# 54rt1n/shardmerge

Measured on AMD Instinct MI355X. Metric: merged-weight GB/s per GPU + % HBM roofline, Llama-3-70B 3-way FFT merge, higher is better.
Workload: dtype f32; 1 GPU; Llama-3-70B block tensors, this rank's 1/8 slice (9 per block x 10 blocks), K=3 finetunes, bf16 in/out, resident in HBM; workload_id=llama3-70b-slice, k=3, parallelism=tensor-partition x1 (no data-path collective), streams_per_gpu=8

## Files before the change

### shardmerge_amd/csrc/fft_engine.hpp

```cpp
#pragma once
#include <cmath>
#include <cstdint>
#include <type_traits>

#if defined(__HIPCC__)
#include <hip/hip_runtime.h>
#define SM_HD __host__ __device__ __forceinline__
#else
#define SM_HD inline
#endif
#define SM_CONST static constexpr
#if defined(__HIP_DEVICE_COMPILE__)
#define SM_OPAQUE(x) asm volatile("" : "+v"(x))
#else
#define SM_OPAQUE(x) ((void)0)
#endif
#if defined(__HIP_DEVICE_COMPILE__)
#define SM_LAUNDER(x) asm("" : "+v"(x))
#else
#define SM_LAUNDER(x) ((void)0)
#endif
#if defined(__HIP_DEVICE_COMPILE__) && !defined(SM_NO_SCHED_BARRIER)
#define SM_SCHED_FENCE() __builtin_amdgcn_sched_barrier(0)
#else
#define SM_SCHED_FENCE() ((void)0)
#endif

namespace smhip {

#include "twiddle_consts.inc"

constexpr int EMAX = 32;
constexpr int EREG = EMAX + 4;
constexpr int MAX_PASSES = 8;

struct cf2 { float x, y; };

#if defined(__HIP_DEVICE_COMPILE__)
typedef float vf2 __attribute__((ext_vector_type(2)));
SM_HD vf2 mk2(float a, float b) { vf2 v; v.x = a; v.y = b; return v; }
#else
struct vf2 { float x, y; };
SM_HD vf2 mk2(float a, float b) { vf2 v; v.x = a; v.y = b; return v; }
SM_HD vf2 operator+(vf2 a, vf2 b) { return mk2(a.x + b.x, a.y + b.y); }
SM_HD vf2 operator-(vf2 a, vf2 b) { return mk2(a.x - b.x, a.y - b.y); }
SM_HD vf2 operator*(vf2 a, vf2 b) { return mk2(a.x * b.x, a.y * b.y); }
SM_HD vf2 operator*(vf2 a, float b) { return mk2(a.x * b, a.y * b); }
SM_HD vf2 operator*(float a, vf2 b) { return mk2(a * b.x, a * b.y); }
SM_HD vf2 operator-(vf2 a) { return mk2(-a.x, -a.y); }
SM_HD vf2& operator+=(vf2& a, vf2 b) { a = a + b; return a; }
#endif

struct FftPlanDev {
    int N;
    int T;
    int npass;
    int radix[MAX_PASSES];
    const cf2* tw;
    int lds_floats;
    int cx;
};

template <int I, int N, class F>
SM_HD void static_for(F&& f) {
    if constexpr (I < N) {
        f(std::integral_constant<int, I>{});
        static_for<I + 1, N>(f);
    }
// ... 661 lines not shown
```

### shardmerge_amd/csrc/sm_capi.inc

```

struct smhip_ctx {
    smhip::Pipeline<SM_BACKEND> pipe;
    explicit smhip_ctx(int device) : pipe(device) {}
};

#define SM_GUARD(ctx)                      \
    if (!(ctx)) return SMHIP_ERR_ARG;      \
    (ctx)->pipe.err.clear();
#define SM_FINISH(ctx, rc)                                                        \
    do {                                                                          \
        int rc__ = (rc);                                                          \
        if (rc__ == SMHIP_OK && !(ctx)->pipe.be.ok()) {                           \
            (ctx)->pipe.err = (ctx)->pipe.be.error();                             \
            rc__ = SMHIP_ERR_HIP;                                                 \
        }                                                                         \
        return rc__;                                                              \
    } while (0)

template <class Desc, class Scalars>
static int delta_tensor_check(smhip_ctx* ctx, const char* op, const Desc* d, const void* out, const float* delta_out,
                              bool need_base, Scalars scalars) {
    auto bad = [&](const char* what) { return ctx->pipe.fail(SMHIP_ERR_ARG, std::string(op) + ": " + what); };
    if (!d) return bad("null descriptor");
    if (d->k < 1 || d->k > SMHIP_MAX_MODELS) return bad("k out of range (1..16)");
// ... 703 lines not shown
    SM_GUARD(ctx);
    if (!norm_out || (n > 0 && !x)) return ctx->pipe.fail(SMHIP_ERR_ARG, "bad argument");
    if (dtype < SMHIP_BF16 || dtype > SMHIP_F32) return ctx->pipe.fail(SMHIP_ERR_ARG, "bad dtype");
    ctx->pipe.stream = stream;
    SM_FINISH(ctx, ctx->pipe.fn_exact_norm(x, dtype, n, norm_out));
}

int smhip_correlate_pairs(smhip_ctx* ctx, int k, const void* const* tensors, int dtype, size_t rows, size_t cols,
                          float* matrix_out, void* stream) {
    SM_GUARD(ctx);
    if (!tensors || !matrix_out || rows < 1 || cols < 1) return ctx->pipe.fail(SMHIP_ERR_ARG, "bad argument");
    if (dtype < SMHIP_BF16 || dtype > SMHIP_F32) return ctx->pipe.fail(SMHIP_ERR_ARG, "bad dtype");
    for (int i = 0; i < k && i < 8; ++i)
        if (!tensors[i]) return ctx->pipe.fail(SMHIP_ERR_ARG, "null tensor");
    ctx->pipe.stream = stream;
    SM_FINISH(ctx, ctx->pipe.correlate_pairs(k, tensors, dtype, rows, cols, matrix_out));
}

int smhip_reference_cpu_norm(smhip_ctx* ctx, const void* x, const void* base, int dtype, size_t n, float* norm_out,
                             void* stream) {
    SM_GUARD(ctx);
    if (!x || !norm_out) return ctx->pipe.fail(SMHIP_ERR_ARG, "bad argument");
    if (dtype < SMHIP_BF16 || dtype > SMHIP_F32) return ctx->pipe.fail(SMHIP_ERR_ARG, "bad dtype");
    ctx->pipe.stream = stream;
    const int rc0 = ctx->pipe.reserve(1, 1);
    if (rc0) SM_FINISH(ctx, rc0);
    smhip::SigDesc sg{x, base, dtype, 1.f};
    double out = 0;
    if (!ctx->pipe.run_serial_norms(&sg, 1, n, &out))
        return ctx->pipe.fail(SMHIP_ERR_ARG, "reference_cpu norm: inputs must be 16-byte aligned");
    *norm_out = (float)out;
    SM_FINISH(ctx, SMHIP_OK);
}

int smhip_debug_option(smhip_ctx* ctx, const char* key, long value) {
    SM_GUARD(ctx);
    if (key && std::string(key) == "aten_overlap") { ctx->pipe.aten_overlap = value != 0; return SMHIP_OK; }
    if (key && std::string(key) == "emf_max_sample") { ctx->pipe.emf_max_sample = value >= 1 && value <= 4096 ? (int)value : smhip::EMF_MAX_SAMPLE; return SMHIP_OK; }
    if (key && std::string(key) == "aten_serial") { ctx->pipe.aten_serial = value != 0; return SMHIP_OK; }
    if (key && std::string(key) == "class_norms") { ctx->pipe.class_norms_mode = value >= 0 && value <= 2 ? (int)value : 1; return SMHIP_OK; }
    if (key && std::string(key) == "cand_cap") { ctx->pipe.debug_cand_cap = value > 0 ? (uint32_t)value : 0u; return SMHIP_OK; }
    if (key && std::string(key) == "sel_chunks") { ctx->pipe.debug_sel_chunks = value > 0 ? (uint32_t)value : 0u; return SMHIP_OK; }
    if (key && std::string(key) == "sel_flush_always") { ctx->pipe.debug_flush_always = value != 0; return SMHIP_OK; }
    if (key && std::string(key) == "fuse_norms") { ctx->pipe.fuse_norms = value != 0; return SMHIP_OK; }
    if (key && std::string(key) == "noise_seed") { ctx->pipe.noise_seed_base = (uint32_t)value; return SMHIP_OK; }
    if (key && std::string(key) == "spectral_intermediates") { ctx->pipe.spectral_inter = value != 0; return SMHIP_OK; }
    if (key && std::string(key) == "fuse_spec_norm") { ctx->pipe.fuse_spec_norm = value != 0; return SMHIP_OK; }
    if (key && std::string(key) == "sel_wgs_per_cu") { ctx->pipe.sel_wgs_per_cu = value > 0 ? (int)value : 5; return SMHIP_OK; }
    if (key && std::string(key) == "pair1d") { ctx->pipe.pair1d_enabled = value != 0; return SMHIP_OK; }
    if (key && std::string(key) == "spec_cull") { ctx->pipe.spec_cull = value != 0; return SMHIP_OK; }
    if (key && std::string(key) == "spec_min_bins") { ctx->pipe.spec_min_bins = value >= 0 ? (size_t)value : (size_t)1 << 20; return SMHIP_OK; }
    if (key && std::string(key) == "dftp_pairs") { ctx->pipe.dftp_pairs_enabled = value != 0; return SMHIP_OK; }
    if (key && std::string(key) == "f2s_pair") { ctx->pipe.f2s_pair = value != 0; return SMHIP_OK; }
    if (key && std::string(key) == "f1_multi") { ctx->pipe.f1_multi = value != 0; return SMHIP_OK; }
    if (key && std::string(key) == "force_bluestein") { ctx->pipe.debug_force_bluestein = value != 0; return SMHIP_OK; }
    if (key && std::string(key) == "force_split") { ctx->pipe.debug_force_split = value > 1 && value <= smhip::DFTP_MAX_P ? (int)value : 0; return SMHIP_OK; }
    if (key && std::string(key) == "fold_columns") { ctx->pipe.fold_enabled = value != 0; return SMHIP_OK; }
    if (key && std::string(key) == "della_slab_rows") { ctx->pipe.delta.della_slab_rows = value > 0 ? (size_t)value : 0; return SMHIP_OK; }
    if (key && std::string(key) == "fold_min_rows") { ctx->pipe.fold_min_rows = value > 0 ? (int)value : SM_FOLD_MIN_ROWS; return SMHIP_OK; }
    return ctx->pipe.fail(SMHIP_ERR_ARG, "unknown debug option");
}

int smhip_debug_query(smhip_ctx* ctx, const char* key, long* value) {
    SM_GUARD(ctx);
    if (!key || !value) return SMHIP_ERR_ARG;
    if (std::string(key) == "spec_hit") { *value = ctx->pipe.last_spec_verdict(); SM_FINISH(ctx, SMHIP_OK); }
    if (std::string(key) == "spec_checked" || std::string(key) == "spec_hits") {
        unsigned long long c = 0, h = 0;
        ctx->pipe.spec_totals(&c, &h);
        *value = (long)(std::string(key) == "spec_hits" ? h : c);
        SM_FINISH(ctx, SMHIP_OK);
    }
    if (std::string(key) == "aten_fast" || std::string(key) == "aten_group" || std::string(key) == "aten_slow") {
        unsigned long long v3[3];
        ctx->pipe.aten_stats(1, v3);
        *value = (long)v3[std::string(key) == "aten_fast" ? 0 : std::string(key) == "aten_group" ? 1 : 2];
        SM_FINISH(ctx, SMHIP_OK);
    }
    if (std::string(key) == "eig_host_us") { *value = (long)ctx->pipe.delta.eig_host_us; SM_FINISH(ctx, SMHIP_OK); }
    return ctx->pipe.fail(SMHIP_ERR_ARG, "unknown debug query");
}

int smhip_profile_enable(smhip_ctx* ctx, int on) { SM_GUARD(ctx); ctx->pipe.be.profile_enable(on != 0); return SMHIP_OK; }
int smhip_profile_reset(smhip_ctx* ctx) { SM_GUARD(ctx); ctx->pipe.be.profile_reset(); return SMHIP_OK; }
int smhip_profile_count(smhip_ctx* ctx) { return ctx ? ctx->pipe.be.profile_count() : 0; }
int smhip_profile_get(smhip_ctx* ctx, int i, const char** name, uint64_t* launches, double* total_ms) {
    SM_GUARD(ctx);
    return ctx->pipe.be.profile_get(i, name, launches, total_ms) ? SMHIP_OK : SMHIP_ERR_ARG;
}

}
```

### shardmerge_amd/csrc/sm_kernels.hpp

```cpp
#pragma once
#include <cmath>
#include <cstring>

#include "fft_engine.hpp"
#include "sm_aten_core.hpp"

namespace smhip {

struct cf4 { float x, y, z, w; };
struct u32x4 { uint32_t x, y, z, w; };

enum { DT_BF16 = 0, DT_F16 = 1, DT_F32 = 2 };

struct SigDesc {
    const void* x;
    const void* base;
    int dtype;
    float prescale;
};

SM_HD uint32_t umax(uint32_t a, uint32_t b) { return a > b ? a : b; }
SM_HD float u2f(uint32_t u) { float f; memcpy(&f, &u, 4); return f; }
SM_HD uint32_t f2u(float f) { uint32_t u; memcpy(&u, &f, 4); return u; }
SM_HD float bf16_to_f(uint32_t h) { return u2f(h << 16); }
// ... 620 lines not shown
                Dft<4>::run(ar, ai);
                Dft<4>::run(br, bi);
#pragma unroll
                for (int k1 = 0; k1 < 4; ++k1) {
                    if (k1) {
                        const cf2 wa = p.twR[(size_t)n2A * k1], wb = p.twR[(size_t)n2B * k1];
                        cmul(ar[k1], ai[k1], wa.x, wa.y); cmul(br[k1], bi[k1], wb.x, wb.y);
                    }
                    cf4 v = {ar[k1], ai[k1], br[k1], bi[k1]};
                    if (live) rowp[(size_t)k * p.ilv + k1 * slabstride] = v;
                }
                SM_SCHED_FENCE();
            };
#pragma unroll
            for (int jj = 0; jj < NJ; ++jj) {
                const int u = 4 * jj + g;
                if (u < E2) {
                    const int k = t + u * T;
                    const int k2 = (k == 0) ? 0 : C - k;
                    float aim[4], bre[4];
#pragma unroll
                    for (int gp = 0; gp < 4; ++gp) {
                        const float* l = lds + gp * LF;
                        const float v1 = l[lpad(k)], v2 = l[lpad(k2)];
                        const int sl = (jj * 4 + gp) * 2;
                        if (comp == 0) { s.xr[sl] = 0.5f * (v1 + v2); s.xr[sl + 1] = 0.5f * (v2 - v1); }
                        else           { aim[gp] = 0.5f * (v1 - v2); bre[gp] = 0.5f * (v1 + v2); }
                    }
                    if (comp == 1) {
                        float are[4], bim[4];
#pragma unroll
                        for (int gp = 0; gp < 4; ++gp) { are[gp] = s.xr[(jj * 4 + gp) * 2]; bim[gp] = s.xr[(jj * 4 + gp) * 2 + 1]; }
                        emit(k, are, aim, bre, bim);
                    }
                }
            }
            if (tid == 0) {
                if (comp == 0) {
#pragma unroll
                    for (int gp = 0; gp < 4; ++gp) s.xr[NJ * 8 + gp] = lds[gp * LF + lpad(C / 2)];
                } else {
                    float are[4], aim[4] = {0.f, 0.f, 0.f, 0.f}, bre[4], bim[4] = {0.f, 0.f, 0.f, 0.f};
#pragma unroll
                    for (int gp = 0; gp < 4; ++gp) { are[gp] = s.xr[NJ * 8 + gp]; bre[gp] = lds[gp * LF + lpad(C / 2)]; }
                    emit(C / 2, are, aim, bre, bim);
                }
            }
        });

    ex.template block_sum<2>(st, [&](const double* tot) {
        partials_[2 * (size_t)pbid] = tot[0];
        partials_[2 * (size_t)pbid + 1] = tot[1];
    });
    }
}

struct SliceGrid { int wgs = 0; size_t t1_stride = 0, plane_stride = 0; };
template <class Ex> SM_HD int slice_of(Ex& ex, const SliceGrid& sl, int& bid) {
    bid = ex.bid();
    if (sl.wgs <= 0) return 0;
    const int s = bid / sl.wgs;
    bid -= s * sl.wgs;
    return s;
}

struct F2Params {
    FftPlanDev plan;
    const cf4* t1;
    int pitch4;
    int ilv;
    int R, C, Cb;
    int nsig;
    int swap;
    float scale[2];
    float* reA; float* imA; float* reB;
    unsigned long long* hist;
    int slab;
    int Cb_real;
    int Rfull;
    size_t slab_elems;
    SliceGrid sl;
};
SM_HD int fold_bin(int v, int slab, int Cb_real, int R2, int Rfull, size_t& off) {
    const int k1 = v / slab, k = v % slab;
    off = (size_t)k * Rfull + (size_t)k1 * R2;
    return k < Cb_real ? k : -1;
}

#ifndef SM_T1_ILV
#define SM_T1_ILV 2
#endif
#ifndef SM_T1_ILV_MIN_ROWS
#define SM_T1_ILV_MIN_ROWS 8192
#endif
#ifndef SM_F2_MAX_THREADS
#define SM_F2_MAX_THREADS 512
#endif
SM_HD constexpr int t1_interleave_rows(int R) { return R >= SM_T1_ILV_MIN_ROWS ? SM_T1_ILV : 1; }
SM_HD constexpr int f2_nsig_for(int T) { return (2 * T <= SM_F2_MAX_THREADS) ? 2 : 1; }

constexpr int FOLD_ILV = 2;
template <class P> constexpr bool fold_col_plan() {
    if constexpr (P::is_static) return f2_nsig_for(P::T) == 2 && (P::N == 2048 || P::N == 3584 || P::N == 4096 || P::N == 7168);
    else return false;
}
template <class P, int BINS, bool FOLD = false, class Ex>
// ... 3167 lines not shown
```

### shardmerge_amd/csrc/sm_pipeline.hpp

```cpp
#pragma once
#include <algorithm>
#include <cmath>
#include <cstdio>
#include <map>
#include <string>
#include <vector>

#include "../../include/shardmerge_hip.h"
#include "sm_kernels.hpp"
#include "sm_aten_norm.hpp"
#include "sm_bluestein.hpp"
#include "sm_lora.hpp"
#include "sm_delta_host.hpp"

namespace smhip {

#define SM_KERNEL_TAG(Tag, ParamsT, NAME, CALL)                                      \
    struct Tag {                                                                     \
        using Params = ParamsT;                                                      \
        static constexpr int waves = 4;                                              \
        static constexpr int max_threads = 1024;                                     \
        static const char* name() { return NAME; }                                   \
        template <class Ex> static SM_HD void run(Ex& ex, const Params& p) { CALL; } \
    };
template <class P, int GROUPS> constexpr int fft_max_threads() {
    if constexpr (P::is_static) return (GROUPS * P::T < 256) ? 256 : (GROUPS * P::T > 1024 ? 1024 : GROUPS * P::T);
    else return 1024;
}
#ifndef SM_W3_MAX_THREADS
#define SM_W3_MAX_THREADS 256
#endif
#define SM_FFT_KERNEL_TAG(Tag, ParamsT, NAME, CALL, GROUPS, WAVES)                   \
    template <class P> struct Tag {                                                  \
        using Params = ParamsT;                                                      \
        static constexpr int waves = (WAVES < 4 && P::is_static && fft_max_threads<P, GROUPS>() <= SM_W3_MAX_THREADS) ? WAVES : 4; \
        static constexpr int max_threads = waves < 4 ? fft_max_threads<P, GROUPS>() : 1024; \
        static const char* name() { return NAME; }                                   \
        template <class Ex> static SM_HD void run(Ex& ex, const Params& p) { CALL; } \
    };
SM_FFT_KERNEL_TAG(KF1, F1Params, "f1_rows_fwd", k_f1<P>(ex, p), 1, 3)
SM_FFT_KERNEL_TAG(KF2, F2Params, "f2_cols_fwd", (k_f2<P, f2_bins<P>()>(ex, p)), 2 * f2_bins<P>(), 4)
SM_FFT_KERNEL_TAG(KI1x1, I1Params, "i1_cols_inv", (k_i1<P, 1>(ex, p)), 1, 4)
SM_FFT_KERNEL_TAG(KI1x2, I1Params, "i1_cols_inv", (k_i1<P, i1_bins<P>()>(ex, p)), i1_bins<P>(), 4)
SM_FFT_KERNEL_TAG(KI2, I2Params, "i2_rows_inv", k_i2<P>(ex, p), 1, 4)
SM_FFT_KERNEL_TAG(KF2S, F2SParams, "f2s_cols_fwd1", (k_f2s<P, f2s_groups<P>()>(ex, p)), f2s_groups<P>(), 4)
SM_FFT_KERNEL_TAG(KF1Q, F1Params, "f1_rows_fwd", k_f1q<P>(ex, p), 4, 4)
SM_FFT_KERNEL_TAG(KF2Q, F2Params, "f2_cols_fwd", (k_f2<P, f2_bins<P>(), true>(ex, p)), 2 * f2_bins<P>(), 4)
SM_FFT_KERNEL_TAG(KF2SQ, F2SParams, "f2s_cols_fwd1", (k_f2s<P, f2s_groups<P>(), true>(ex, p)), f2s_groups<P>(), 4)
SM_FFT_KERNEL_TAG(KI1x1Q, I1Params, "i1_cols_inv", (k_i1<P, 1, true>(ex, p)), 1, 4)
SM_FFT_KERNEL_TAG(KI1x2Q, I1Params, "i1_cols_inv", (k_i1<P, i1_bins<P>(), true>(ex, p)), i1_bins<P>(), 4)
#define SM_BLUE_KERNEL_TAG(Tag, ParamsT, NAME, CALL)                                 \
    template <class P> struct Tag {                                                  \
        using Params = ParamsT;                                                      \
        static constexpr int max_threads = fft_max_threads<P, 1>();                  \
        static constexpr int waves = max_threads > 512 ? 4 : 2;                      \
        static const char* name() { return NAME; }                                   \
        template <class Ex> static SM_HD void run(Ex& ex, const Params& p) { CALL; } \
    };
SM_BLUE_KERNEL_TAG(KF1B, F1BParams, "f1_rows_fwd", k_f1b<P>(ex, p))
SM_BLUE_KERNEL_TAG(KI2B, I2BParams, "i2_rows_inv", k_i2b<P>(ex, p))
SM_FFT_KERNEL_TAG(KPair1d, Pair1dParams, "pair_1d", k_pair1d<P>(ex, p), 1, 1)

#ifndef SM_COLS_MAX_THREADS
#define SM_COLS_MAX_THREADS 1024
#endif
#ifndef SM_F2_MAX_THREADS
#define SM_F2_MAX_THREADS 512
#endif
#ifndef SM_R14336
#define SM_R14336 16, 16, 8, 7
#endif
#ifndef SM_R7168
#define SM_R7168 32, 32, 7
#endif
#ifndef SM_T8192
#define SM_T8192 256
#define SM_W8192 4
#define SM_R8192 32, 16, 16
#endif
#define SM_STATIC_PLANS(X)                 \
    X(SPlan<1024, 64, false, 4, 32, 32>)       \
    X(SPlan<2048, 64, false, 4, 16, 16, 8>)    \
    X(SPlan<4096, 128, false, 4, 16, 16, 16>)  \
    X(SPlan<8192, SM_T8192, false, SM_W8192, SM_R8192>)  \
    X(SPlan<16384, 512, false, 4, 32, 32, 16>)\
    X(SPlan<14336, 512, false, 4, SM_R14336>) \
    X(SPlan<28672, 1024, false, 4, 16, 16, 16, 7>) \
    X(SPlan<3072, 128, false, 4, 16, 16, 4, 3>)    \
    X(SPlan<3584, 128, false, 4, 16, 32, 7>)       \
    X(SPlan<5120, 256, false, 4, 16, 16, 4, 5>)    \
    X(SPlan<6144, 256, false, 4, 16, 16, 8, 3>)    \
    X(SPlan<7168, 256, false, 4, SM_R7168>)    \
    X(SPlan<12288, 512, false, 4, 16, 16, 16, 3>)  \
    X(SPlan<13824, 512, false, 4, 32, 16, 3, 3, 3>) \
    X(SPlan<27648, 1024, false, 4, 32, 32, 3, 3, 3>) \
    X(SPlan<2304, 128, false, 4, 16, 16, 3, 3>) \
    X(SPlan<256, 64, false, 4, 8, 8, 4>)            \
    X(SPlan<512, 64, false, 4, 32, 16>)             \
    X(SPlan<64, 64, false, 4, 8, 8>)                \
// ... 147 lines not shown
        if (N % p) continue;
        M = N / p;
        if (M % 2 == 0 && plan_shape(M, T, rad)) return true;
    }
    return false;
}
inline int bluestein_len(int C) {
    if (C < 2) return 0;
    for (int L = 256; L <= EMAX * 1024; L *= 2)
        if (L >= 2 * C - 1) return L;
    return 0;
}
inline int shape_support(int rows, int cols, bool* transposed = nullptr) {
    int T, p, M;
    std::vector<int> rad;
    if (transposed) *transposed = false;
    if (rows < 1 || cols < 1) return 0;
    if (plan_shape(cols, T, rad) && rough_split(rows, p, M)) return 1;
    if (plan_shape(rows, T, rad) && rough_split(cols, p, M)) { if (transposed) *transposed = true; return 1; }
    if (bluestein_len(cols) && rough_split(rows, p, M)) return 1;
    if (bluestein_len(rows) && rough_split(cols, p, M)) { if (transposed) *transposed = true; return 1; }
    return 0;
}

struct ProfEntry { std::string name; uint64_t launches = 0; double ms = 0; };

struct PairOut {
    void* out = nullptr; int out_mode = OUT_F32;
    const void* base = nullptr; int base_dtype = DT_BF16;
    float post = 1.f;
    int ifft_policy = 1;
};

template <class B>
class Pipeline {
  public:
    B be;
    std::string err;
    void* stream = nullptr;
    DeltaHost<B> delta{be, err, stream};
    uint32_t debug_cand_cap = 0;
    uint32_t debug_sel_chunks = 0;
    bool debug_flush_always = false;
    bool spec_cull = true;
    size_t spec_min_bins = 1 << 20;
    bool dftp_pairs_enabled = true;
    int debug_force_split = 0;
    int sel_wgs_per_cu = 5;
    bool safe_select = false;
    uint32_t noise_seed_base = 0;
    bool spectral_inter = true;
    bool f2s_pair = true;
    size_t f2s_pair_max_bins = (size_t)64 << 20;
    bool f1_multi = true;
    bool fuse_spec_norm = true;
    float noise_sigma = 1.2e-7f;

    explicit Pipeline(int device) : be(device) {}
    ~Pipeline() {
        for (auto& kv : plans_) if (kv.second.dev.tw) be.free((void*)kv.second.dev.tw);
        for (Buffer* b : {&cand_, &t1_, &small_, &tmpA_, &tmpB_, &tmpC_, &fullS_, &saveR_, &saveI_, &aten_, &emf_, &lora_, &dora_}) if (b->p) be.free(b->p);
        for (Buffer& b : pool_) if (b.p) be.free(b.p);
        if (mail_) be.free_host(mail_);
        for (Buffer& b : inter_) if (b.p) be.free(b.p);
        for (Buffer& b : rowspec_) if (b.p) be.free(b.p);
        for (Buffer& b : tr_) if (b.p) be.free(b.p);
        for (auto& kv : rough_tw_) if (kv.second) be.free(kv.second);
        for (auto& kv : blue_) { if (kv.second.chirp) be.free(kv.second.chirp); if (kv.second.filt) be.free(kv.second.filt); }
    }

    int fail(int code, const std::string& msg) { err = msg; return code; }

    int get_plan(int N, FftPlanDev& out) {
        auto it = plans_.find(N);
        if (it == plans_.end()) {
            HostPlan hp;
            int T;
            std::vector<int> rad;
            if (plan_shape(N, T, rad)) {
                hp.ok = true;
                hp.dev.N = N; hp.dev.T = T; hp.dev.npass = (int)rad.size();
                for (int i = 0; i < MAX_PASSES; ++i) hp.dev.radix[i] = i < (int)rad.size() ? rad[i] : 1;
                hp.dev.cx = plan_uses_cx(N) ? 1 : 0;
                hp.dev.lds_floats = hp.dev.cx ? (int)round_up((size_t)2 * (N + (N >> 4) + 1), 32)
                                              : (int)round_up((size_t)lpad(N) + 1, 32);
                std::vector<cf2> tw(N);
                for (int j = 0; j < N; ++j) {
                    const double ang = -2.0 * M_PI * (double)j / (double)N;
                    tw[j].x = (float)cos(ang); tw[j].y = (float)sin(ang);
                }
                void* d = be.alloc(sizeof(cf2) * N);
                if (!d) return fail(SMHIP_ERR_NOMEM, "twiddle alloc failed");
                be.h2d(d, tw.data(), sizeof(cf2) * N, stream);
                hp.dev.tw = (const cf2*)d;
            } else {
                hp.dev.tw = nullptr;
            }
            it = plans_.emplace(N, hp).first;
        }
        if (!it->second.ok) {
            char buf[256];
            snprintf(buf, sizeof buf, "unsupported transform length %d (a row length needs factors in {2,3,5,7,11,13} and <= %d; the layer merge "
                                       "also takes p * M column lengths, p <= %d)", N, EMAX * 1024, DFTP_MAX_P);
            return fail(SMHIP_ERR_SHAPE, buf);
        }
        out = it->second.dev;
// ... 201 lines not shown
            bh.filt = be.alloc(sizeof(cf2) * L);
            if (!bh.chirp || !bh.filt) return fail(SMHIP_ERR_NOMEM, "chirp table alloc failed");
            be.h2d(bh.chirp, chirp.data(), sizeof(cf2) * C, stream);
            be.h2d(bh.filt, filt.data(), sizeof(cf2) * L, stream);
            be.sync(stream);
            it = blue_.emplace(C, bh).first;
        }
        out.chirp = (const cf2*)it->second.chirp; out.filt = (const cf2*)it->second.filt;
        return SMHIP_OK;
    }
    int get_row_plan(int C, FftPlanDev& plan, bool& blue, BluesteinTab& bt) {
        blue = row_bluestein(C);
        bt.chirp = nullptr; bt.filt = nullptr;
        return blue ? bluestein_tables(C, bt, plan) : get_plan(C, plan);
    }

    int rough_twiddles(int N, const cf2** out) {
        auto it = rough_tw_.find(N);
        if (it == rough_tw_.end()) {
            std::vector<cf2> tw(N);
            for (int j = 0; j < N; ++j) {
                const double ang = -2.0 * M_PI * (double)j / (double)N;
                tw[j].x = (float)cos(ang); tw[j].y = (float)sin(ang);
            }
            void* d = be.alloc(sizeof(cf2) * N);
            if (!d) return fail(SMHIP_ERR_NOMEM, "twiddle alloc failed");
            be.h2d(d, tw.data(), sizeof(cf2) * N, stream);
            be.sync(stream);
            it = rough_tw_.emplace(N, d).first;
        }
        *out = (const cf2*)it->second;
        return SMHIP_OK;
    }
    int run_dftp(const Geo& g, void* buf, bool rowpair, int ilv, int pitch, size_t slice_stride, bool inverse) {
        DftpParams q;
        int rc = rough_twiddles(g.R * g.rough, &q.tw);
        if (rc) return rc;
        q.buf = (cf4*)buf; q.p = g.rough; q.M = g.R; q.units = rowpair ? g.R / 2 : g.R; q.rowpair = rowpair ? 1 : 0;
        q.ilv = ilv; q.pitch = pitch; q.ncols = g.C / 2 + 1; q.slice_stride = slice_stride; q.inverse = inverse ? 1 : 0;
        q.cols = DFTP_COLS;
        if (q.p <= DFTP_PAIR_MAX_P && dftp_pairs_enabled) {
            q.cols = dftp_pairs_cols(q.p);
            const int ntp = (q.ncols + q.cols - 1) / q.cols;
            const size_t ldsp = LDS_SCRATCH_FLOATS * 4 + dftp_pairs_lds_bytes(q.p) + ((size_t)(q.p / 2 + 1) + 64) * sizeof(cf2);
            be.template launch<KDftpPairs>((q.units + DFTP_UNITS - 1) / DFTP_UNITS * ntp, 256, ldsp, q, stream);
            return SMHIP_OK;
        }
        const int ntiles = (q.ncols + DFTP_COLS - 1) / DFTP_COLS;
        const size_t lds = LDS_SCRATCH_FLOATS * 4 + (size_t)q.p * DFTP_COLS * sizeof(cf4) + (size_t)q.p * sizeof(cf2);
        be.template launch<KDftp>(q.units * ntiles, 256, lds, q, stream);
        return SMHIP_OK;
    }

    int run_f1(const Geo& g, const SigDesc& a, const SigDesc& b, int& grid_out) {
        F1Params p;
        bool blue; BluesteinTab bt;
        int rc = get_row_plan(g.C, p.plan, blue, bt);
        if (rc) return rc;
        p.a = a; p.b = b; p.R = g.R; p.C = g.C; p.Cb = g.C / 2 + 1; p.pitch4 = g.pitch4; p.ilv = g.ilv;
        p.sigs.n = 0;
        p.fuse.prefix = nullptr; p.fuse.grp = nullptr; p.fuse.nchunks = 0; p.fuse.sig0 = 0; p.fuse_rowpair = 0;
        p.nb = blue ? 1 : std::max(1, 256 / p.plan.T);
        p.row_stride = (size_t)g.C;
        p.vec = !blue && (g.C % 8 == 0) && aligned16(a.x) && aligned16(a.base) && aligned16(b.x) && aligned16(b.base);
        if (fused_.armed && p.vec && g.batch == 1 && g.rough == 1) { p.fuse = fused_.af; p.fuse_rowpair = 0; fused_.used = true; }
        p.t1 = (cf4*)t1_.p;
        p.partials = d_part();
        p.R2 = 0; p.rowpair = 0; p.Rcol = g.R; p.twR = nullptr; p.slab_elems = fold_slab_elems(g);
        if (g.fold == 4) {
            if (!p.vec) return fail(SMHIP_ERR_ARG, "internal: folded row pass on unaligned input");
            FftPlanDev colp;
            if ((rc = get_plan(g.R, colp))) return rc;
            p.R2 = g.R / 4; p.twR = colp.tw; p.ilv = FOLD_ILV; p.nb = 4;
            const int gridq = (int)round_up((size_t)p.R2, 8 * p.ilv);
            if ((size_t)gridq * 2 > PART_DOUBLES) return fail(SMHIP_ERR_SHAPE, "too many rows");
            launch_fft<KF1Q>(p.plan, gridq, 4 * p.plan.T, (LDS_SCRATCH_FLOATS + (size_t)4 * p.plan.lds_floats) * 4, p);
            grid_out = gridq;
            return SMHIP_OK;
        }
        const int xg = p.ilv > p.nb ? p.ilv / p.nb : 1;
        const bool joint = joint_rows(g);
        const int nlaunch = joint ? 1 : g.batch;
        if (joint) p.R = g.R * g.rough;
        const int grid = (int)round_up((size_t)(p.R + p.nb - 1) / p.nb, 8 * xg);
        if ((size_t)grid * 2 * nlaunch > PART_DOUBLES) return fail(SMHIP_ERR_SHAPE, "too many rows");
        const size_t lds = (LDS_SCRATCH_FLOATS + (size_t)p.nb * p.plan.lds_floats) * 4;
        for (int bi = 0; bi < nlaunch; ++bi) {
            p.a = sig_at(a, (size_t)bi * g.R * g.C); p.b = sig_at(b, (size_t)bi * g.R * g.C);
            p.t1 = (cf4*)t1_.p + (size_t)bi * g.t1_slice;
            p.partials = d_part() + (size_t)bi * 2 * grid;
            if (blue) { F1BParams q; q.f = p; q.bt = bt; launch_fft<KF1B>(p.plan, grid, p.plan.T, lds, q); }
            else launch_fft<KF1>(p.plan, grid, p.nb * p.plan.T, lds, p, p.vec != 0);
        }
        grid_out = grid * nlaunch;
        if (g.rough > 1) return run_dftp(g, t1_.p, false, p.ilv, g.pitch4, g.t1_slice, false);
        return SMHIP_OK;
    }
    static size_t dt_size(int dt) { return dt == DT_F32 ? 4 : 2; }
    static SigDesc sig_at(const SigDesc& s, size_t elems) {
        SigDesc r = s;
        if (r.x) r.x = (const char*)r.x + elems * dt_size(s.dtype);
        if (r.base) r.base = (const char*)r.base + elems * dt_size(s.dtype);
        return r;
    }
    static size_t fold_slab_elems(const Geo& g, bool rowpair = false) {
        return round_up((size_t)g.R / (rowpair ? 8 : 4), 8) * (size_t)g.pitch4;
    }
    static bool joint_rows(const Geo& g) { return g.rough > 1 && g.R % 16 == 0; }
    int run_f1_rowpairs(const Geo& g, const SigDesc& sig, void* t1buf = nullptr, double* partials = nullptr, int* grid_out = nullptr,
                        F1Sigs* multi = nullptr) {
        F1Params p;
        bool blue; BluesteinTab bt;
        int rc = get_row_plan(g.C, p.plan, blue, bt);
        if (rc) return rc;
        SigDesc a = sig, b = sig;
        b.x = (const char*)sig.x + (size_t)g.C * dt_size(sig.dtype);
        if (sig.base) b.base = (const char*)sig.base + (size_t)g.C * dt_size(sig.dtype);
        p.a = a; p.b = b; p.R = g.R / 2; p.C = g.C; p.Cb = g.C / 2 + 1; p.pitch4 = g.pitch4; p.ilv = F2S_ILV;
        p.sigs.n = 0;
        p.fuse.prefix = nullptr; p.fuse.grp = nullptr; p.fuse.nchunks = 0; p.fuse.sig0 = 0; p.fuse_rowpair = 0;
        const int nm = multi ? multi->n : 1;
        if (multi && (blue || nm < 2 || nm > F1_MAX_SIGS)) return SMHIP_ERR_ARG;
        p.nb = blue ? 1 : std::max(1, 256 / p.plan.T);
        p.row_stride = (size_t)2 * g.C;
        p.vec = !blue && (g.C % 8 == 0) && aligned16(a.x) && aligned16(a.base) && aligned16(b.x) && aligned16(b.base);
        if (fused_.armed && p.vec && g.batch == 1 && g.rough == 1) {
            p.fuse = fused_.af; p.fuse.sig0 = multi ? 0 : fused_.next_sig; p.fuse_rowpair = 1; fused_.used = true;
        }
        p.t1 = (cf4*)(t1buf ? t1buf : t1_.p);
        p.partials = partials ? partials : d_part();
        p.R2 = 0; p.rowpair = 0; p.Rcol = g.R; p.twR = nullptr; p.slab_elems = fold_slab_elems(g, true);
        if (g.fold == 4) {
            if (!p.vec) return fail(SMHIP_ERR_ARG, "internal: folded row pass on unaligned input");
            FftPlanDev colp;
            if ((rc = get_plan(g.R, colp))) return rc;
            p.R2 = g.R / 8; p.rowpair = 1; p.twR = colp.tw; p.ilv = F2S_ILV; p.nb = 4;
            const int gridq = (int)round_up((size_t)p.R2, 8 * p.ilv);
            if (multi) {
                if ((size_t)gridq * 2 * nm > PART_DOUBLES) return SMHIP_ERR_ARG;
                for (int i = 0; i < nm; ++i) multi->partials[i] = p.partials + (size_t)i * 2 * gridq;
                multi->b_off = (long long)((size_t)g.C * dt_size(sig.dtype));
                p.sigs = *multi;
            }
            launch_fft<KF1Q>(p.plan, gridq * nm, 4 * p.plan.T, (LDS_SCRATCH_FLOATS + (size_t)4 * p.plan.lds_floats) * 4, p);
            if (grid_out) *grid_out = gridq;
            return SMHIP_OK;
        }
        const int xgs = p.ilv > p.nb ? p.ilv / p.nb : 1;
        const bool joint = joint_rows(g);
        const int nlaunch = joint ? 1 : g.batch;
        if (joint) p.R = g.R * g.rough / 2;
        const int grid = (int)round_up((size_t)(p.R + p.nb - 1) / p.nb, 8 * xgs);
        if (multi && (nlaunch != 1 || g.rough > 1 || (size_t)grid * 2 * nm > PART_DOUBLES || !p.vec)) return SMHIP_ERR_ARG;
        if ((size_t)grid * 2 * nlaunch > PART_DOUBLES) return fail(SMHIP_ERR_SHAPE, "too many rows");
        const size_t lds = (LDS_SCRATCH_FLOATS + (size_t)p.nb * p.plan.lds_floats) * 4;
        cf4* const t1base = p.t1;
        double* const pbase = p.partials;
        if (multi) {
            for (int i = 0; i < nm; ++i) multi->partials[i] = pbase + (size_t)i * 2 * grid;
            multi->b_off = (long long)((size_t)g.C * dt_size(sig.dtype));
            p.sigs = *multi;
            launch_fft<KF1>(p.plan, grid * nm, p.nb * p.plan.T, lds, p, true);
            if (grid_out) *grid_out = grid;
            return SMHIP_OK;
        }
        for (int bi = 0; bi < nlaunch; ++bi) {
            p.a = sig_at(a, (size_t)bi * g.R * g.C); p.b = sig_at(b, (size_t)bi * g.R * g.C);
            p.t1 = t1base + (size_t)bi * (g.t1_slice / 2);
            p.partials = pbase + (size_t)bi * 2 * grid;
            if (blue) { F1BParams q; q.f = p; q.bt = bt; launch_fft<KF1B>(p.plan, grid, p.plan.T, lds, q); }
            else launch_fft<KF1>(p.plan, grid, p.nb * p.plan.T, lds, p, p.vec != 0);
        }
        if (grid_out) *grid_out = grid * nlaunch;
        if (g.rough > 1) return run_dftp(g, t1base, true, F2S_ILV, g.pitch4, g.t1_slice / 2, false);
        return SMHIP_OK;
    }
    struct F2SSecond { const void* t1; bool role_a; float scale; };
    int run_f2s(const Geo& g, bool role_a, float scale, bool hist, const void* t1buf = nullptr, int* im_parts = nullptr,
                const F2SSecond* second = nullptr) {
        F2SParams p;
        p.two = 0; p.t1_2 = nullptr; p.role_a_2 = 0; p.scale_2 = 0.f; p.re_2 = nullptr;
        if (second) {
            if (g.batch != 1 || second->role_a == role_a) return fail(SMHIP_ERR_ARG, "internal: paired column pass");
            p.two = 1; p.t1_2 = (const cf4*)second->t1; p.role_a_2 = second->role_a ? 1 : 0; p.scale_2 = second->scale;
            p.re_2 = plane(g, second->role_a ? P_REA : P_REB);
        }
        const int nsg = second ? 2 : 1;
        const int Rt = g.R / g.fold;
        int rc = get_plan(Rt, p.plan);
        if (rc) return rc;
        p.t1 = (const cf4*)(t1buf ? t1buf : t1_.p); p.pitch4 = g.pitch4 * g.fold; p.R = Rt; p.C = g.C;
        p.Cb = g.fold == 4 ? 4 * g.pitch4 : g.C / 2 + 1;
        p.slab = g.pitch4; p.Cb_real = g.C / 2 + 1; p.Rfull = g.R; p.slab_elems = fold_slab_elems(g, true);
        p.role_a = role_a ? 1 : 0; p.scale = scale;
        p.re = plane(g, role_a ? P_REA : P_REB); p.im = plane(g, P_IMA);
        p.hist = hist ? d_hist() : nullptr;
        const bool st = is_static_plan(p.plan);
// ... 1693 lines not shown
```

### shardmerge_amd/csrc/smhip_device.hpp

```cpp
#pragma once
#include <hip/hip_runtime.h>

#include "sm_pipeline.hpp"

namespace smhip {

struct DeviceExec {
    template <class S> struct State { using value_type = S; S s; };
    __device__ __forceinline__ int bid() const { return blockIdx.x; }
    __device__ __forceinline__ int nthreads() const { return blockDim.x; }
    __device__ __forceinline__ int nblocks() const { return gridDim.x; }
    __device__ __forceinline__ float* lds() {
        extern __shared__ __attribute__((aligned(16))) float sm_dyn_lds[];
        return sm_dyn_lds;
    }
    template <class S> __device__ __forceinline__ void init(State<S>&) {}
    template <class S, class F> __device__ __forceinline__ void each(State<S>& st, F&& f) { f((int)threadIdx.x, st.s); }
    __device__ __forceinline__ void sync() { __syncthreads(); }
    __device__ __forceinline__ void lds_atomic_add(uint32_t* p, uint32_t v) { atomicAdd(p, v); }
    __device__ __forceinline__ uint32_t lds_atomic_add_ret(uint32_t* p, uint32_t v) { return atomicAdd(p, v); }
    __device__ __forceinline__ uint32_t global_atomic_add_ret_u32(uint32_t* p, uint32_t v) { return atomicAdd(p, v); }
    __device__ __forceinline__ void global_atomic_add(unsigned long long* p, unsigned long long v) { atomicAdd(p, v); }
    __device__ __forceinline__ void global_atomic_add_u32(uint32_t* p, uint32_t v) { atomicAdd(p, v); }
    __device__ __forceinline__ void global_atomic_or_u32(uint32_t* p, uint32_t v) { atomicOr(p, v); }
// ... 6 lines not shown
        for (int i = 0; i < N; ++i) b[i] = (uint32_t)__shfl_down((int)a[i], DELTA, 64);
    }
    template <int NP, class S, class Get>
    __device__ __forceinline__ void lane_pair_trade(State<S>& st, Get get) {
        const bool odd = (threadIdx.x & 1u) != 0;
        static_for<0, NP>([&](auto k_c) {
            auto pr = get(st.s, k_c);
            const float give = odd ? pr.a : pr.b;
            const float got = __builtin_bit_cast(float, __builtin_amdgcn_mov_dpp(__builtin_bit_cast(int, give), 0xB1, 0xF, 0xF, true));
            pr.a = odd ? got : pr.a;
            pr.b = odd ? pr.b : got;
        });
    }
    template <int NV, class S, class F>
    __device__ __forceinline__ void block_sum(State<S>& st, F&& f) {
        double v[NV];
#pragma unroll
        for (int q = 0; q < NV; ++q) v[q] = st.s.red[q];
#pragma unroll
        for (int off = 32; off > 0; off >>= 1) {
#pragma unroll
            for (int q = 0; q < NV; ++q) v[q] += __shfl_down(v[q], off, 64);
        }
        double* scratch = (double*)lds();
        const int wave = threadIdx.x >> 6, lane = threadIdx.x & 63;
        const int nw = (blockDim.x + 63) >> 6;
        if (lane == 0) {
#pragma unroll
            for (int q = 0; q < NV; ++q) scratch[wave * NV + q] = v[q];
        }
        __syncthreads();
        if (threadIdx.x == 0) {
            double tot[NV];
#pragma unroll
            for (int q = 0; q < NV; ++q) tot[q] = 0.0;
            for (int w = 0; w < nw; ++w) {
#pragma unroll
                for (int q = 0; q < NV; ++q) tot[q] += scratch[w * NV + q];
            }
            f((const double*)tot);
        }
        __syncthreads();
    }
};

template <class K>
__global__ void __launch_bounds__(K::max_threads, K::waves) sm_kernel(const typename K::Params p) {
    DeviceExec ex;
    K::run(ex, p);
}

#define SM_FFT_KERNELS_OF(X, ...)                      \
    X(KF1<__VA_ARGS__>) X(KF2<__VA_ARGS__>) X(KI1x1<__VA_ARGS__>) X(KI1x2<__VA_ARGS__>) X(KI2<__VA_ARGS__>) X(KF2S<__VA_ARGS__>) \
    X(KF1Q<__VA_ARGS__>) X(KF2Q<__VA_ARGS__>) X(KF2SQ<__VA_ARGS__>) X(KI1x1Q<__VA_ARGS__>) X(KI1x2Q<__VA_ARGS__>) \
    X(KPair1d<__VA_ARGS__>) X(KF1B<__VA_ARGS__>) X(KI2B<__VA_ARGS__>)

}
```

### shardmerge_amd/csrc/smhip_side.hip

```cpp
#include "smhip_device.hpp"

namespace smhip {
#define SM_INST(...) template __global__ void sm_kernel<__VA_ARGS__>(const typename __VA_ARGS__::Params);
#if SM_SIDE_GROUP == 0
SM_SIDE_KERNELS_0(SM_INST)
#elif SM_SIDE_GROUP == 1
SM_SIDE_KERNELS_1(SM_INST)
#elif SM_SIDE_GROUP == 2
SM_SIDE_KERNELS_2(SM_INST)
#elif SM_SIDE_GROUP == 3
SM_INST(KF1<DynPlan>) SM_INST(KF1Q<DynPlan>) SM_INST(KI2<DynPlan>) SM_INST(KPair1d<DynPlan>)
#elif SM_SIDE_GROUP == 4
SM_INST(KF2<DynPlan>) SM_INST(KF2Q<DynPlan>) SM_INST(KF2S<DynPlan>) SM_INST(KF2SQ<DynPlan>)
#elif SM_SIDE_GROUP == 5
SM_INST(KI1x1<DynPlan>) SM_INST(KI1x2<DynPlan>) SM_INST(KI1x1Q<DynPlan>) SM_INST(KI1x2Q<DynPlan>)
#elif SM_SIDE_GROUP == 6
SM_INST(KF1B<DynPlan>) SM_INST(KI2B<DynPlan>)
#elif SM_SIDE_GROUP == 7
SM_SIDE_KERNELS_7(SM_INST)
#elif SM_SIDE_GROUP == 8
SM_SIDE_KERNELS_8(SM_INST)
#elif SM_SIDE_GROUP == 9
SM_SIDE_KERNELS_9(SM_INST)
#elif SM_SIDE_GROUP == 10
SM_SIDE_KERNELS_10(SM_INST)
#elif SM_SIDE_GROUP == 11
SM_SIDE_KERNELS_11(SM_INST)
#elif SM_SIDE_GROUP == 12
SM_SIDE_KERNELS_12(SM_INST)
#elif SM_SIDE_GROUP == 13
SM_SIDE_KERNELS_13(SM_INST)
#elif SM_SIDE_GROUP == 14
SM_SIDE_KERNELS_14(SM_INST)
#elif SM_SIDE_GROUP == 15
SM_SIDE_KERNELS_15(SM_INST)
#elif SM_SIDE_GROUP == 16
SM_SIDE_KERNELS_16(SM_INST)
#else
#error "SM_SIDE_GROUP must be 0..16"
#endif
}
```

Baseline: 86.78 GB/s.

## Split folded row-FFT kernel into two half-workgroups per row quad

Adds a KF1H kernel that splits the 4-row folded forward row FFT across two workgroups, each computing one half of the radix-4 fold (k1 even pair or odd pair) using two FFT groups instead of four. The grid doubles, while LDS and thread count per workgroup halve. The aim is better occupancy and a shorter per-workgroup critical path on the first FFT stage. In exchange, each half re-reads all four input rows, so input loads are duplicated, and only half 0 writes the norm partials. It is enabled by default through the f1q_halves option.

```diff
diff --git a/shardmerge_amd/csrc/fft_engine.hpp b/shardmerge_amd/csrc/fft_engine.hpp
--- a/shardmerge_amd/csrc/fft_engine.hpp
+++ b/shardmerge_amd/csrc/fft_engine.hpp
@@ -14,6 +14,12 @@
 #define SM_OPAQUE(x) asm volatile("" : "+v"(x))
 #else
 #define SM_OPAQUE(x) ((void)0)
+#endif
+#define SM_LAMBDA_INLINE __attribute__((always_inline))
+#if defined(__HIP_DEVICE_COMPILE__)
+#define SM_WAVE_UNIFORM(x) ((x) = __builtin_amdgcn_readfirstlane(x))
+#else
+#define SM_WAVE_UNIFORM(x) ((void)0)
 #endif
 #if defined(__HIP_DEVICE_COMPILE__)
 #define SM_LAUNDER(x) asm("" : "+v"(x))
diff --git a/shardmerge_amd/csrc/sm_capi.inc b/shardmerge_amd/csrc/sm_capi.inc
--- a/shardmerge_amd/csrc/sm_capi.inc
+++ b/shardmerge_amd/csrc/sm_capi.inc
@@ -779,6 +779,7 @@
     if (key && std::string(key) == "spec_min_bins") { ctx->pipe.spec_min_bins = value >= 0 ? (size_t)value : (size_t)1 << 20; return SMHIP_OK; }
     if (key && std::string(key) == "dftp_pairs") { ctx->pipe.dftp_pairs_enabled = value != 0; return SMHIP_OK; }
     if (key && std::string(key) == "f2s_pair") { ctx->pipe.f2s_pair = value != 0; return SMHIP_OK; }
+    if (key && std::string(key) == "f1q_halves") { ctx->pipe.f1q_halves = value != 0; return SMHIP_OK; }
     if (key && std::string(key) == "f1_multi") { ctx->pipe.f1_multi = value != 0; return SMHIP_OK; }
     if (key && std::string(key) == "force_bluestein") { ctx->pipe.debug_force_bluestein = value != 0; return SMHIP_OK; }
     if (key && std::string(key) == "force_split") { ctx->pipe.debug_force_split = value > 1 && value <= smhip::DFTP_MAX_P ? (int)value : 0; return SMHIP_OK; }
diff --git a/shardmerge_amd/csrc/sm_kernels.hpp b/shardmerge_amd/csrc/sm_kernels.hpp
--- a/shardmerge_amd/csrc/sm_kernels.hpp
+++ b/shardmerge_amd/csrc/sm_kernels.hpp
@@ -696,6 +696,239 @@
         partials_[2 * (size_t)pbid] = tot[0];
         partials_[2 * (size_t)pbid + 1] = tot[1];
     });
+    }
+}
+
+struct F1HState {
+    float xr[EREG];
+    float xi[EREG];
+    double red[4];
+};
+
+template <class P, class Ex>
+SM_HD void k_f1h(Ex& ex, const F1Params& p) {
+    if constexpr (!f1q_eligible<P>()) { return; } else {
+    typename Ex::template State<F1HState> st;
+    ex.init(st);
+    float* lds = ex.lds() + LDS_SCRATCH_FLOATS;
+    const FftPlanDev& pl = p.plan;
+    constexpr int T = P::T, C = P::N, LF = P::lds_floats;
+    constexpr int E2 = C / T / 2;
+    constexpr int NJ = (E2 + 1) / 2;
+    constexpr int NQ = EMAX / 8;
+    static_assert(NJ * 4 + 2 <= EREG, "register slots");
+    const int nsig = p.sigs.n > 1 ? p.sigs.n : 1;
+    int s2_;
+    const int unit = pick_signal(2 * nsig, ex.bid(), p.ilv > 1 ? p.ilv : 1, s2_);
+    const int sig_ = s2_ >> 1, half = s2_ & 1;
+    SigDesc sa = p.a, sb = p.b;
+    cf4* t1_ = p.t1;
+    double* partials_ = p.partials;
+    if (p.sigs.n > 1) {
+        sa.x = p.sigs.x[sig_]; sa.base = p.sigs.base[sig_];
+        sb.x = (const char*)sa.x + p.sigs.b_off; sb.base = sa.base ? (const char*)sa.base + p.sigs.b_off : nullptr;
+        t1_ = p.sigs.t1[sig_]; partials_ = p.sigs.partials[sig_];
+    }
+    const bool live = unit < p.R2;
+    const bool bits16 = sa.dtype != DT_F32 && sb.dtype != DT_F32;
+    const bool has_b = sb.x != nullptr;
+    const int n2A = !live ? 0 : p.rowpair ? 2 * unit : unit, n2B = !live ? 0 : p.rowpair ? 2 * unit + 1 : unit;
+    const int k1lo = half, k1hi = 2 + half;
+    cf4* const rowp = t1_ + (size_t)(unit / p.ilv) * p.pitch4 * p.ilv + (unit % p.ilv);
+    const size_t slabstride = p.slab_elems;
+
+    ex.each(st, [&](int, F1HState& s) { s.red[0] = 0.0; s.red[1] = 0.0; });
+
+    wg_fft<P, SM_F1Q_PACK, 1>(ex, st, pl, lds,
+        [&](int tid, F1HState& s, auto comp_c) {
+            constexpr int comp = decltype(comp_c)::value;
+            int tid_ = tid;
+            SM_OPAQUE(tid_);
+            int g = tid_ >= T ? 1 : 0;
+            SM_WAVE_UNIFORM(g);
+            const int t = tid_ - g * T;
+            float* l = lds + g * LF;
+            if constexpr (comp == 1) {
+#pragma unroll
+                for (int q = 0; q < NQ; ++q) {
+                    const int n0 = 8 * (t + q * T);
+                    if (n0 < C) {
+#pragma unroll
+                        for (int c = 0; c < 8; ++c) l[lpad(n0 + c)] = s.xi[q * 8 + c];
+                    }
+                }
+            } else {
+                const bool have = g == 0 || has_b;
+                const bool useb = g != 0 && has_b;
+                const void* const ax = sa.x; const void* const bx = sb.x;
+                const void* const abase = sa.base; const void* const bbase = sb.base;
+                const int adt = sa.dtype, bdt = sb.dtype;
+                const float asc = sa.prescale, bsc = sb.prescale;
+                const void* const gx = useb ? bx : ax;
+                const void* const gbase = useb ? bbase : abase;
+                const int gdt = useb ? bdt : adt;
+                const float gscale = useb ? bsc : asc;
+                const bool has_base = gbase != nullptr;
+                double ss = 0.0;
+                auto finish = [&](auto q_c, bool ok, float (&x)[4][8]) SM_LAMBDA_INLINE {
+                    constexpr int q = decltype(q_c)::value;
+                    const int n0 = 8 * (t + q * T);
+#pragma unroll
+                    for (int r = 0; r < 4; ++r) {
+                        float qs = 0.f;
+#pragma unroll
+                        for (int c = 0; c < 8; ++c) {
+                            if (!ok || !have) x[r][c] = 0.f;
+                            qs += x[r][c] * x[r][c];
+                        }
+                        ss += qs;
+                    }
+#pragma unroll
+                    for (int c = 0; c < 8; ++c) {
+                        float re, im;
+                        if (half == 0) {
+                            const float e = x[0][c] + x[2][c], o = x[1][c] + x[3][c];
+                            re = e + o; im = e - o;
+                        } else {
+                            re = x[0][c] - x[2][c]; im = x[1][c] - x[3][c];
+                        }
+                        l[lpad(n0 + c)] = re;
+                        s.xi[q * 8 + c] = im;
+                    }
+                };
+                auto offs = [&](int q, bool& ok, size_t* off) SM_LAMBDA_INLINE {
+                    const int n0 = 8 * (t + q * T);
+                    ok = live && n0 < C;
+#pragma unroll
+                    for (int r = 0; r < 4; ++r) off[r] = ok ? (size_t)(unit + r * p.R2) * p.row_stride + n0 : (size_t)0;
+                };
+                auto rows16 = [&](auto dt_c) SM_LAMBDA_INLINE {
+                    constexpr int DT = decltype(dt_c)::value;
+                    const u32x4* px = (const u32x4*)gx;
+                    const u32x4* pb = has_base ? (const u32x4*)gbase : px;
+                    static_for<0, NQ>([&](auto q_c) {
+                        constexpr int q = decltype(q_c)::value;
+                        if (8 * (t + q * T) < C) {
+                            SM_SCHED_FENCE();
+                            bool ok; size_t off[4];
+                            offs(q, ok, off);
+                            u32x4 rx[4], rb[4];
+#pragma unroll
+                            for (int r = 0; r < 4; ++r) rx[r] = px[off[r] / 8];
+#pragma unroll
+                            for (int r = 0; r < 4; ++r) rb[r] = pb[off[r] / 8];
+                            float x[4][8];
+#pragma unroll
+                            for (int r = 0; r < 4; ++r) {
+                                float bv[8];
+                                decode16x8(rx[r], DT, x[r]);
+                                decode16x8(rb[r], DT, bv);
+#pragma unroll
+                                for (int c = 0; c < 8; ++c) x[r][c] = (x[r][c] - (has_base ? bv[c] : 0.f)) * gscale;
+                            }
+                            finish(q_c, ok, x);
+                            SM_SCHED_FENCE();
+                        }
+                    });
+                };
+                if (bits16 && gdt == DT_BF16) rows16(std::integral_constant<int, DT_BF16>{});
+                else if (bits16) rows16(std::integral_constant<int, DT_F16>{});
+                else {
+                    SigDesc sg;
+                    sg.x = gx; sg.base = gbase; sg.dtype = gdt; sg.prescale = gscale;
+                    static_for<0, NQ>([&](auto q_c) {
+                        constexpr int q = decltype(q_c)::value;
+                        if (8 * (t + q * T) < C) {
+                            SM_SCHED_FENCE();
+                            bool ok; size_t off[4];
+                            offs(q, ok, off);
+                            float x[4][8];
+#pragma unroll
+                            for (int r = 0; r < 4; ++r) load_sig8(sg, off[r], x[r]);
+                            finish(q_c, ok, x);
+                            SM_SCHED_FENCE();
+                        }
+                    });
+                }
+                if (g == 0) s.red[0] += ss; else s.red[1] += ss;
+            }
+        },
+        [&](int tid, F1HState& s, auto comp_c) {
+            constexpr int comp = decltype(comp_c)::value;
+            int tid_ = tid;
+            SM_OPAQUE(tid_);
+            int g = tid_ >= T ? 1 : 0;
+            SM_WAVE_UNIFORM(g);
+            const int t = tid_ - g * T;
+            auto emit = [&](int k, const float* fre, const float* fim, const float* gre, const float* gim) SM_LAMBDA_INLINE {
+                SM_SCHED_FENCE();
+                float lr[2], li[2], hr[2], hi[2];
+#pragma unroll
+                for (int sl = 0; sl < 2; ++sl) {
+                    if (half == 0) { lr[sl] = fre[sl]; li[sl] = fim[sl]; hr[sl] = gre[sl]; hi[sl] = gim[sl]; }
+                    else {
+                        lr[sl] = fre[sl] + gim[sl]; li[sl] = fim[sl] - gre[sl];
+                        hr[sl] = fre[sl] - gim[sl]; hi[sl] = fim[sl] + gre[sl];
+                    }
+                }
+                if (half != 0) {
+                    const cf2 wa = p.twR[(size_t)n2A * k1lo], wb = p.twR[(size_t)n2B * k1lo];
+                    cmul(lr[0], li[0], wa.x, wa.y); cmul(lr[1], li[1], wb.x, wb.y);
+                }
+                {
+                    const cf2 wa = p.twR[(size_t)n2A * k1hi], wb = p.twR[(size_t)n2B * k1hi];
+                    cmul(hr[0], hi[0], wa.x, wa.y); cmul(hr[1], hi[1], wb.x, wb.y);
+                }
+                if (!has_b) { lr[1] = 0.f; li[1] = 0.f; hr[1] = 0.f; hi[1] = 0.f; }
+                if (live) {
+                    const cf4 vlo = {lr[0], li[0], lr[1], li[1]}, vhi = {hr[0], hi[0], hr[1], hi[1]};
+                    rowp[(size_t)k * p.ilv + k1lo * slabstride] = vlo;
+                    rowp[(size_t)k * p.ilv + k1hi * slabstride] = vhi;
+                }
+                SM_SCHED_FENCE();
+            };
+#pragma unroll
+            for (int jj = 0; jj < NJ; ++jj) {
+                const int u = 2 * jj + g;
+                if (u < E2) {
+                    const int k = t + u * T;
+                    const int k2 = (k == 0) ? 0 : C - k;
+                    float fim[2], gre[2];
+#pragma unroll
+                    for (int sl = 0; sl < 2; ++sl) {
+                        const float* l = lds + sl * LF;
+                        const float v1 = l[lpad(k)], v2 = l[lpad(k2)];
+                        const int ix = (jj * 2 + sl) * 2;
+                        if (comp == 0) { s.xr[ix] = 0.5f * (v1 + v2); s.xr[ix + 1] = 0.5f * (v2 - v1); }
+                        else           { fim[sl] = 0.5f * (v1 - v2); gre[sl] = 0.5f * (v1 + v2); }
+                    }
+                    if (comp == 1) {
+                        float fre[2], gim[2];
+#pragma unroll
+                        for (int sl = 0; sl < 2; ++sl) { fre[sl] = s.xr[(jj * 2 + sl) * 2]; gim[sl] = s.xr[(jj * 2 + sl) * 2 + 1]; }
+                        emit(k, fre, fim, gre, gim);
+                    }
+                }
+            }
+            if (tid == 0) {
+                if (comp == 0) {
+#pragma unroll
+                    for (int sl = 0; sl < 2; ++sl) s.xr[NJ * 4 + sl] = lds[sl * LF + lpad(C / 2)];
+                } else {
+                    float fre[2], fim[2] = {0.f, 0.f}, gre[2], gim[2] = {0.f, 0.f};
+#pragma unroll
+                    for (int sl = 0; sl < 2; ++sl) { fre[sl] = s.xr[NJ * 4 + sl]; gre[sl] = lds[sl * LF + lpad(C / 2)]; }
+                    emit(C / 2, fre, fim, gre, gim);
+                }
+            }
+        });
+
+    if (half == 0) {
+        ex.template block_sum<2>(st, [&](const double* tot) {
+            partials_[2 * (size_t)unit] = tot[0];
+            partials_[2 * (size_t)unit + 1] = tot[1];
+        });
+    }
     }
 }
 
diff --git a/shardmerge_amd/csrc/sm_pipeline.hpp b/shardmerge_amd/csrc/sm_pipeline.hpp
--- a/shardmerge_amd/csrc/sm_pipeline.hpp
+++ b/shardmerge_amd/csrc/sm_pipeline.hpp
@@ -45,6 +45,7 @@
 SM_FFT_KERNEL_TAG(KI2, I2Params, "i2_rows_inv", k_i2<P>(ex, p), 1, 4)
 SM_FFT_KERNEL_TAG(KF2S, F2SParams, "f2s_cols_fwd1", (k_f2s<P, f2s_groups<P>()>(ex, p)), f2s_groups<P>(), 4)
 SM_FFT_KERNEL_TAG(KF1Q, F1Params, "f1_rows_fwd", k_f1q<P>(ex, p), 4, 4)
+SM_FFT_KERNEL_TAG(KF1H, F1Params, "f1_rows_fwd", k_f1h<P>(ex, p), 2, 4)
 SM_FFT_KERNEL_TAG(KF2Q, F2Params, "f2_cols_fwd", (k_f2<P, f2_bins<P>(), true>(ex, p)), 2 * f2_bins<P>(), 4)
 SM_FFT_KERNEL_TAG(KF2SQ, F2SParams, "f2s_cols_fwd1", (k_f2s<P, f2s_groups<P>(), true>(ex, p)), f2s_groups<P>(), 4)
 SM_FFT_KERNEL_TAG(KI1x1Q, I1Params, "i1_cols_inv", (k_i1<P, 1, true>(ex, p)), 1, 4)
@@ -298,6 +299,7 @@
     bool spectral_inter = true;
     bool f2s_pair = true;
     size_t f2s_pair_max_bins = (size_t)64 << 20;
+    bool f1q_halves = true;
     bool f1_multi = true;
     bool fuse_spec_norm = true;
     float noise_sigma = 1.2e-7f;
@@ -605,6 +607,10 @@
         return SMHIP_OK;
     }
 
+    void launch_f1_folded(const F1Params& p, int units) {
+        if (f1q_halves) launch_fft<KF1H>(p.plan, units * 2, 2 * p.plan.T, (LDS_SCRATCH_FLOATS + (size_t)2 * p.plan.lds_floats) * 4, p);
+        else launch_fft<KF1Q>(p.plan, units, 4 * p.plan.T, (LDS_SCRATCH_FLOATS + (size_t)4 * p.plan.lds_floats) * 4, p);
+    }
     int run_f1(const Geo& g, const SigDesc& a, const SigDesc& b, int& grid_out) {
         F1Params p;
         bool blue; BluesteinTab bt;
@@ -627,7 +633,7 @@
             p.R2 = g.R / 4; p.twR = colp.tw; p.ilv = FOLD_ILV; p.nb = 4;
             const int gridq = (int)round_up((size_t)p.R2, 8 * p.ilv);
             if ((size_t)gridq * 2 > PART_DOUBLES) return fail(SMHIP_ERR_SHAPE, "too many rows");
-            launch_fft<KF1Q>(p.plan, gridq, 4 * p.plan.T, (LDS_SCRATCH_FLOATS + (size_t)4 * p.plan.lds_floats) * 4, p);
+            launch_f1_folded(p, gridq);
             grid_out = gridq;
             return SMHIP_OK;
         }
@@ -695,7 +701,7 @@
                 multi->b_off = (long long)((size_t)g.C * dt_size(sig.dtype));
                 p.sigs = *multi;
             }
-            launch_fft<KF1Q>(p.plan, gridq * nm, 4 * p.plan.T, (LDS_SCRATCH_FLOATS + (size_t)4 * p.plan.lds_floats) * 4, p);
+            launch_f1_folded(p, gridq * nm);
             if (grid_out) *grid_out = gridq;
             return SMHIP_OK;
         }
diff --git a/shardmerge_amd/csrc/smhip_device.hpp b/shardmerge_amd/csrc/smhip_device.hpp
--- a/shardmerge_amd/csrc/smhip_device.hpp
+++ b/shardmerge_amd/csrc/smhip_device.hpp
@@ -82,7 +82,7 @@
 
 #define SM_FFT_KERNELS_OF(X, ...)                      \
     X(KF1<__VA_ARGS__>) X(KF2<__VA_ARGS__>) X(KI1x1<__VA_ARGS__>) X(KI1x2<__VA_ARGS__>) X(KI2<__VA_ARGS__>) X(KF2S<__VA_ARGS__>) \
-    X(KF1Q<__VA_ARGS__>) X(KF2Q<__VA_ARGS__>) X(KF2SQ<__VA_ARGS__>) X(KI1x1Q<__VA_ARGS__>) X(KI1x2Q<__VA_ARGS__>) \
+    X(KF1Q<__VA_ARGS__>) X(KF1H<__VA_ARGS__>) X(KF2Q<__VA_ARGS__>) X(KF2SQ<__VA_ARGS__>) X(KI1x1Q<__VA_ARGS__>) X(KI1x2Q<__VA_ARGS__>) \
     X(KPair1d<__VA_ARGS__>) X(KF1B<__VA_ARGS__>) X(KI2B<__VA_ARGS__>)
 
 }
diff --git a/shardmerge_amd/csrc/smhip_side.hip b/shardmerge_amd/csrc/smhip_side.hip
--- a/shardmerge_amd/csrc/smhip_side.hip
+++ b/shardmerge_amd/csrc/smhip_side.hip
@@ -9,7 +9,7 @@
 #elif SM_SIDE_GROUP == 2
 SM_SIDE_KERNELS_2(SM_INST)
 #elif SM_SIDE_GROUP == 3
-SM_INST(KF1<DynPlan>) SM_INST(KF1Q<DynPlan>) SM_INST(KI2<DynPlan>) SM_INST(KPair1d<DynPlan>)
+SM_INST(KF1<DynPlan>) SM_INST(KF1Q<DynPlan>) SM_INST(KF1H<DynPlan>) SM_INST(KI2<DynPlan>) SM_INST(KPair1d<DynPlan>)
 #elif SM_SIDE_GROUP == 4
 SM_INST(KF2<DynPlan>) SM_INST(KF2Q<DynPlan>) SM_INST(KF2S<DynPlan>) SM_INST(KF2SQ<DynPlan>)
 #elif SM_SIDE_GROUP == 5
```

New measurement: 86.96 GB/s, median of 6. About the same (+0.2%).
